# zkonduit/ezkl

Hardware: NVIDIA H100
Metric: prove_time_s (lower is better)
Workload: dtype u32 limbs (254-bit Montgomery integers mod BN254 r/p)

## Files before the change

ezkl_b200/csrc/msm.cu:

```cuda
#include "msm.cuh"
#include "ec_coop.cuh"

namespace b200 {

static constexpr int HEAVY_CHUNKS = 32;
static constexpr int REDUCE_M_MAX = 32;
static constexpr int TREE_THREADS = 256;

int msm_default_window(size_t n) {
    int k = 0;
    while (((size_t)1 << (k + 1)) <= n) ++k;
    int c = k <= 10 ? 8 : (k <= 13 ? k - 2 : (k <= 17 ? k - 1 : (k <= 19 ? 17 : (k <= 21 ? 18 : 20))));
    if (c < 4) c = 4;
    if (c > 22) c = 22;
    return c;
}

__global__ void __launch_bounds__(128) k_table_next_level(const G1Affine* __restrict__ prev, G1Affine* __restrict__ next, size_t n, int c) {
    size_t i = (size_t)blockIdx.x * blockDim.x + threadIdx.x;
    if (i >= n) return;
    G1Affine p = prev[i];
    G1Xyzz a = g1_dbl_affine(p);
#pragma unroll 1
    for (int j = 1; j < c; ++j) a = g1_dbl(a);
    next[i] = g1_to_affine(a);
}

int msm_table_build(MsmTable* t, const G1Affine* d_bases, size_t n, int c, cudaStream_t st) {
    B200_CHECK(n > 0, -1, "msm_table_build: empty base vector");
    if (c <= 0) c = msm_default_window(n);
    int W = (255 + c - 1) / c;
    B200_CHECK((size_t)W * n < ((size_t)1 << 31), -1, "msm_table_build: W*n = %zu exceeds the 31-bit entry index", (size_t)W * n);
    t->n = n; t->c = c; t->W = W;
    B200_CUDA(cudaGetDevice(&t->device));
    B200_CUDA(cudaMalloc(&t->d_table, sizeof(G1Affine) * n * W));
    B200_CUDA(cudaMemcpyAsync(t->d_table, d_bases, sizeof(G1Affine) * n, cudaMemcpyDeviceToDevice, st));
    for (int w = 1; w < W; ++w) {
        k_table_next_level<<<div_up(n, 128), 128, 0, st>>>(t->d_table + (size_t)(w - 1) * n, t->d_table + (size_t)w * n, n, c); count_launch();
    }
    B200_CUDA(cudaGetLastError());
    return 0;
}
void msm_table_free(MsmTable* t) {
    if (t->d_table) cudaFree(t->d_table);
    t->d_table = nullptr;
}

template <bool SCATTER>
__global__ void __launch_bounds__(256) k_digits(const Fr* __restrict__ scalars, size_t stride, uint32_t n, uint32_t table_n, uint32_t base_off, int c, int W,
                                                 uint32_t nbuckets, uint32_t* __restrict__ counters ,
                                                 const uint32_t* __restrict__ offs , uint32_t* __restrict__ ents, size_t ent_stride,
                                                 const uint32_t* __restrict__ skew) {
    const uint32_t col = blockIdx.y;
    const bool aggregate = !SCATTER || skew[col] != 0;
    const Fr* sc = scalars + (size_t)col * stride;
    uint32_t* cnt = counters + (size_t)col * nbuckets;
    const uint32_t* off = SCATTER ? offs + (size_t)col * (nbuckets + 1) : nullptr;
    uint32_t* ent = SCATTER ? ents + (size_t)col * ent_stride : nullptr;
    const unsigned lane = threadIdx.x & 31;
    const uint32_t n_up = (n + 31u) & ~31u;
    for (uint32_t i = blockIdx.x * blockDim.x + threadIdx.x; i < n_up; i += gridDim.x * blockDim.x) {
        const bool valid = i < n;
        Fr s = fp_zero<FrTag>();
        if (valid) s = fp_from_mont(fp_load(sc + i));
        uint32_t carry = 0;
#pragma unroll 1
        for (int w = 0; w < W; ++w) {
            int32_t d = msm_next_digit(s.l, c, &carry);
            const bool nz = d != 0;
            const unsigned act = __ballot_sync(0xffffffffu, nz);
            if (nz && !aggregate) {
                const uint32_t bucket = (uint32_t)(d < 0 ? -d : d) - 1u;
                ent[off[bucket] + atomicAdd(&cnt[bucket], 1u)] = ((uint32_t)w * table_n + base_off + i) | (d < 0 ? 0x80000000u : 0u);
            } else if (nz) {
                const uint32_t bucket = (uint32_t)(d < 0 ? -d : d) - 1u;
                const unsigned peers = __match_any_sync(act, bucket);
                const int leader = __ffs(peers) - 1;
                uint32_t base = 0;
                if ((int)lane == leader) base = atomicAdd(&cnt[bucket], (uint32_t)__popc(peers));
                if (SCATTER) {
                    base = __shfl_sync(peers, base, leader);
                    const uint32_t rank = __popc(peers & ((1u << lane) - 1u));
                    ent[off[bucket] + base + rank] = ((uint32_t)w * table_n + base_off + i) | (d < 0 ? 0x80000000u : 0u);
                }
            }
        }
    }
}

__global__ void __launch_bounds__(1024) k_scan_buckets(const uint32_t* __restrict__ counts, uint32_t* __restrict__ offs, uint32_t* __restrict__ chunk_offs,
                                                        uint32_t nbuckets, uint32_t cap, uint32_t* __restrict__ skew ) {
    __shared__ uint32_t sh_max;
    if (threadIdx.x == 0) sh_max = 0;
    __syncthreads();
    const uint32_t col = blockIdx.x;
    const uint32_t lc = 31u - (uint32_t)__clz(cap);
    const uint32_t* cnt = counts + (size_t)col * nbuckets;
    uint32_t* off = offs + (size_t)col * (nbuckets + 1);
    uint32_t* coff = chunk_offs + (size_t)col * (nbuckets + 1);
    const uint32_t ipt = (nbuckets + blockDim.x - 1) / blockDim.x;
    const uint32_t lo = threadIdx.x * ipt, hi = min(lo + ipt, nbuckets);
    uint32_t s = 0, cs = 0;
    uint32_t mx = 0;
    const bool vec = (ipt & 3u) == 0 && lo + ipt <= nbuckets;
    if (vec) {
        const uint4* c4 = reinterpret_cast<const uint4*>(cnt + lo);
#pragma unroll 4
        for (uint32_t q = 0; q < (ipt >> 2); ++q) {
            const uint4 v = c4[q];
            s += v.x + v.y + v.z + v.w;
            cs += ((v.x + cap - 1) >> lc) + ((v.y + cap - 1) >> lc) + ((v.z + cap - 1) >> lc) + ((v.w + cap - 1) >> lc);
            mx = max(max(mx, v.x), max(max(v.y, v.z), v.w));
        }
    } else {
        for (uint32_t b = lo; b < hi; ++b) { uint32_t v = cnt[b]; s += v; cs += ((v + cap - 1) >> lc); mx = max(mx, v); }
    }
    if (mx) atomicMax(&sh_max, mx);
    uint32_t tot, ctot;
    uint32_t ex = block_exclusive_scan(s, &tot);
    uint32_t cex = block_exclusive_scan(cs, &ctot);
    if (vec) {
        const uint4* c4 = reinterpret_cast<const uint4*>(cnt + lo);
#pragma unroll 4
        for (uint32_t q = 0; q < (ipt >> 2); ++q) {
            const uint4 v = c4[q];
            const uint32_t b = lo + 4 * q;
            off[b] = ex; coff[b] = cex; ex += v.x; cex += ((v.x + cap - 1) >> lc);
            off[b + 1] = ex; coff[b + 1] = cex; ex += v.y; cex += ((v.y + cap - 1) >> lc);
            off[b + 2] = ex; coff[b + 2] = cex; ex += v.z; cex += ((v.z + cap - 1) >> lc);
            off[b + 3] = ex; coff[b + 3] = cex; ex += v.w; cex += ((v.w + cap - 1) >> lc);
        }
    } else {
        for (uint32_t b = lo; b < hi; ++b) { uint32_t v = cnt[b]; off[b] = ex; coff[b] = cex; ex += v; cex += ((v + cap - 1) >> lc); }
    }
    if (threadIdx.x == 0) {
        off[nbuckets] = tot; coff[nbuckets] = ctot;
        skew[col] = sh_max > 16u * (tot / nbuckets + 1u) ? 1u : 0u;
    }
}

__global__ void __launch_bounds__(256) k_fill_chunks(const uint32_t* __restrict__ offs, const uint32_t* __restrict__ chunk_offs, uint32_t nbuckets, uint32_t cap,
                                                      uint32_t* __restrict__ chunk_start, uint32_t* __restrict__ chunk_len, size_t chunk_stride,
                                                      uint32_t* __restrict__ len_hist , uint32_t* __restrict__ heavy , uint32_t heavy_stride) {
    extern __shared__ uint32_t sh_hist[];
    const uint32_t col = blockIdx.y;
    for (uint32_t j = threadIdx.x; j <= cap; j += blockDim.x) sh_hist[j] = 0;
    __syncthreads();
    const uint32_t* off = offs + (size_t)col * (nbuckets + 1);
    const uint32_t* coff = chunk_offs + (size_t)col * (nbuckets + 1);
    uint32_t* cs = chunk_start + (size_t)col * chunk_stride;
    uint32_t* cl = chunk_len + (size_t)col * chunk_stride;
    const uint32_t b = blockIdx.x * blockDim.x + threadIdx.x;
    if (b < nbuckets) {
        const uint32_t start = off[b], size = off[b + 1] - start, c0 = coff[b], nch = coff[b + 1] - c0;
        for (uint32_t j = 0; j < nch; ++j) {
            const uint32_t len = min(cap, size - j * cap);
            cs[c0 + j] = start + j * cap;
            cl[c0 + j] = len;
            if (j + 1 == nch) atomicAdd(&sh_hist[len], 1u);
        }
        if (nch > 1) atomicAdd(&sh_hist[cap], nch - 1);
        if (nch > (uint32_t)HEAVY_CHUNKS) {
            uint32_t* hv = heavy + (size_t)col * heavy_stride;
            uint32_t slot = atomicAdd(&hv[0], 1u);
            if (slot + 1 < heavy_stride) hv[1 + slot] = b;
        }
    }
    __syncthreads();
    uint32_t* gh = len_hist + (size_t)col * (cap + 1);
    for (uint32_t j = threadIdx.x; j <= cap; j += blockDim.x) if (sh_hist[j]) atomicAdd(&gh[j], sh_hist[j]);
}

__global__ void k_len_offsets(const uint32_t* __restrict__ len_hist, uint32_t* __restrict__ len_offs, uint32_t cap) {
    const uint32_t col = blockIdx.x;
    if (threadIdx.x != 0) return;
    const uint32_t* h = len_hist + (size_t)col * (cap + 1);
    uint32_t* o = len_offs + (size_t)col * (cap + 1);
    uint32_t acc = 0;
    for (int l = (int)cap; l >= 0; --l) { o[l] = acc; acc += h[l]; }
}

__global__ void __launch_bounds__(256) k_order_chunks(const uint32_t* __restrict__ chunk_len, size_t chunk_stride, const uint32_t* __restrict__ chunk_offs, uint32_t nbuckets,
                                                       const uint32_t* __restrict__ len_offs, uint32_t* __restrict__ len_cursor, uint32_t cap, uint32_t* __restrict__ order) {
    const uint32_t col = blockIdx.y;
    const uint32_t nchunks = chunk_offs[(size_t)col * (nbuckets + 1) + nbuckets];
    const uint32_t* cl = chunk_len + (size_t)col * chunk_stride;
    uint32_t* ord = order + (size_t)col * chunk_stride;
    const uint32_t* lo = len_offs + (size_t)col * (cap + 1);
    uint32_t* lc = len_cursor + (size_t)col * (cap + 1);
    const unsigned lane = threadIdx.x & 31;
    const uint32_t n_up = (nchunks + 31u) & ~31u;
    for (uint32_t i = blockIdx.x * blockDim.x + threadIdx.x; i < n_up; i += gridDim.x * blockDim.x) {
        const bool valid = i < nchunks;
        const uint32_t len = valid ? cl[i] : 0;
        const unsigned act = __ballot_sync(0xffffffffu, valid);
        if (valid) {
            const unsigned peers = __match_any_sync(act, len);
            const int leader = __ffs(peers) - 1;
            uint32_t base = 0;
            if ((int)lane == leader) base = atomicAdd(&lc[len], (uint32_t)__popc(peers));
            base = __shfl_sync(peers, base, leader);
            ord[lo[len] + base + __popc(peers & ((1u << lane) - 1u))] = i;
        }
    }
}

DEV G1Affine load_base(const G1Affine* __restrict__ table, uint32_t e) {
    const uint4* q = reinterpret_cast<const uint4*>(table + (e & 0x7fffffffu));
    uint4 a = __ldg(q), b = __ldg(q + 1), c = __ldg(q + 2), d = __ldg(q + 3);
    G1Affine p;
    p.x.l[0] = a.x; p.x.l[1] = a.y; p.x.l[2] = a.z; p.x.l[3] = a.w; p.x.l[4] = b.x; p.x.l[5] = b.y; p.x.l[6] = b.z; p.x.l[7] = b.w;
    p.y.l[0] = c.x; p.y.l[1] = c.y; p.y.l[2] = c.z; p.y.l[3] = c.w; p.y.l[4] = d.x; p.y.l[5] = d.y; p.y.l[6] = d.z; p.y.l[7] = d.w;
    return p;
}
__global__ void __launch_bounds__(128, 4) k_accumulate(const G1Affine* __restrict__ table, const uint32_t* __restrict__ ents, size_t ent_stride,
                                                        const uint32_t* __restrict__ chunk_start, const uint32_t* __restrict__ chunk_len, const uint32_t* __restrict__ order,
                                                        size_t chunk_stride, const uint32_t* __restrict__ chunk_offs, uint32_t nbuckets, G1Xyzz* __restrict__ chunk_sums) {
    const uint32_t col = blockIdx.y;
    const uint32_t nchunks = chunk_offs[(size_t)col * (nbuckets + 1) + nbuckets];
    const uint32_t* ent = ents + (size_t)col * ent_stride;
    for (uint32_t t = blockIdx.x * blockDim.x + threadIdx.x; t < nchunks; t += gridDim.x * blockDim.x) {
        const uint32_t ch = order[(size_t)col * chunk_stride + t];
        const uint32_t start = chunk_start[(size_t)col * chunk_stride + ch], len = chunk_len[(size_t)col * chunk_stride + ch];
        uint32_t e = ent[start];
        G1Affine p = load_base(table, e);
        if (e >> 31) p = g1_neg(p);
        G1Xyzz acc = g1_to_xyzz(p);
        if (len > 1) {
            uint32_t e_next = ent[start + 1];
            G1Affine nx = load_base(table, e_next);
#pragma unroll 1
            for (uint32_t j = 1; j < len; ++j) {
                p = nx; e = e_next;
                if (j + 1 < len) { e_next = ent[start + j + 1]; nx = load_base(table, e_next); }
                if (e >> 31) p = g1_neg(p);
                acc = g1_add_mixed(acc, p);
            }
        }
        chunk_sums[(size_t)col * chunk_stride + ch] = acc;
    }
}

DEV G1Xyzz block_sum(G1Xyzz v, G1Xyzz* sh) {
    sh[threadIdx.x] = v;
    __syncthreads();
#pragma unroll 1
    for (unsigned s = blockDim.x / 2; s > 0; s >>= 1) {
        if (threadIdx.x < s) { v = g1_add(v, sh[threadIdx.x + s]); sh[threadIdx.x] = v; }
        __syncthreads();
    }
    return v;
}

__global__ void __launch_bounds__(128) k_combine(const uint32_t* __restrict__ chunk_offs, uint32_t nbuckets, const G1Xyzz* __restrict__ chunk_sums, size_t chunk_stride,
                                                  G1Xyzz* __restrict__ bucket_sums) {
    const uint32_t col = blockIdx.y;
    const uint32_t b = blockIdx.x * blockDim.x + threadIdx.x;
    if (b >= nbuckets) return;
    const uint32_t* coff = chunk_offs + (size_t)col * (nbuckets + 1);
    const uint32_t c0 = coff[b], nch = coff[b + 1] - c0;
    if (nch > (uint32_t)HEAVY_CHUNKS) return;
    const G1Xyzz* cs = chunk_sums + (size_t)col * chunk_stride;
    G1Xyzz acc = g1_xyzz_identity();
    if (nch > 0) acc = cs[c0];
#pragma unroll 1
    for (uint32_t j = 1; j < nch; ++j) acc = g1_add(acc, cs[c0 + j]);
    bucket_sums[(size_t)col * nbuckets + b] = acc;
}
__global__ void __launch_bounds__(TREE_THREADS) k_combine_heavy(const uint32_t* __restrict__ heavy, uint32_t heavy_stride, const uint32_t* __restrict__ chunk_offs, uint32_t nbuckets,
                                                                 const G1Xyzz* __restrict__ chunk_sums, size_t chunk_stride, G1Xyzz* __restrict__ bucket_sums) {
    __shared__ G1Xyzz sh[TREE_THREADS];
    const uint32_t col = blockIdx.y;
    const uint32_t* hv = heavy + (size_t)col * heavy_stride;
    const uint32_t nheavy = min(hv[0], heavy_stride - 1);
    const uint32_t* coff = chunk_offs + (size_t)col * (nbuckets + 1);
    const G1Xyzz* cs = chunk_sums + (size_t)col * chunk_stride;
    for (uint32_t h = blockIdx.x; h < nheavy; h += gridDim.x) {
        const uint32_t b = hv[1 + h];
        const uint32_t c0 = coff[b], nch = coff[b + 1] - c0;
        G1Xyzz acc = g1_xyzz_identity();
#pragma unroll 1
        for (uint32_t j = threadIdx.x; j < nch; j += TREE_THREADS) acc = g1_add(acc, cs[c0 + j]);
        acc = block_sum(acc, sh);
        if (threadIdx.x == 0) bucket_sums[(size_t)col * nbuckets + b] = acc;
        __syncthreads();
    }
}

template <int MIN_CTAS>
__global__ void __launch_bounds__(TREE_THREADS, MIN_CTAS) k_reduce(const G1Xyzz* __restrict__ bucket_sums, uint32_t nbuckets, G1Xyzz* __restrict__ partials, uint32_t nparts, uint32_t per_thread) {
    __shared__ G1Xyzz sh[TREE_THREADS];
    const uint32_t col = blockIdx.y;
    const G1Xyzz* bs = bucket_sums + (size_t)col * nbuckets;
    const uint32_t t = blockIdx.x * blockDim.x + threadIdx.x;
    const uint32_t lo = t * per_thread;
    G1Xyzz run = g1_xyzz_identity(), acc = g1_xyzz_identity();
    if (lo < nbuckets) {
        const uint32_t hi = min(lo + per_thread, nbuckets);
#pragma unroll 1
        for (uint32_t b = hi; b-- > lo;) {
            run = g1_add(run, bs[b]);
            acc = g1_add(acc, run);
        }
        if (lo > 0) acc = g1_add(acc, g1_mul_small(run, lo));
    }
    acc = block_sum(acc, sh);
    if (threadIdx.x == 0) partials[(size_t)col * nparts + blockIdx.x] = acc;
}
__global__ void __launch_bounds__(TREE_THREADS) k_final(const G1Xyzz* __restrict__ partials, uint32_t nparts, G1Xyzz* __restrict__ out) {
    __shared__ G1Xyzz sh[TREE_THREADS];
    const uint32_t col = blockIdx.x;
    G1Xyzz acc = g1_xyzz_identity();
#pragma unroll 1
    for (uint32_t j = threadIdx.x; j < nparts; j += blockDim.x) acc = g1_add(acc, partials[(size_t)col * nparts + j]);
    acc = block_sum(acc, sh);
    if (threadIdx.x == 0) out[col] = acc;
}

static constexpr int COOP_LT = TREE_THREADS / 4;
static constexpr size_t COOP_MAX_BUCKETS = (size_t)3 << 15;
DEV G1Xyzz block_sum_coop(G1Xyzz v, G1Xyzz* sh) {
    const unsigned lt = threadIdx.x >> 2, q = threadIdx.x & 3;
    if (q == 0) sh[lt] = v;
    __syncthreads();
#pragma unroll 1
    for (unsigned s = COOP_LT / 2; s > 0; s >>= 1) {
        if (lt < s) { v = g1_add_coop4(v, sh[lt + s]); if (q == 0) sh[lt] = v; }
        __syncthreads();
    }
    return v;
}
__global__ void __launch_bounds__(TREE_THREADS) k_reduce_coop(const G1Xyzz* __restrict__ bucket_sums, uint32_t nbuckets, G1Xyzz* __restrict__ partials, uint32_t nparts, uint32_t per_thread) {
    __shared__ G1Xyzz sh[COOP_LT];
    const uint32_t col = blockIdx.y;
    const G1Xyzz* bs = bucket_sums + (size_t)col * nbuckets;
    const uint32_t t = blockIdx.x * COOP_LT + (threadIdx.x >> 2);
    const uint32_t lo = t * per_thread;
    G1Xyzz run = g1_xyzz_identity(), acc = g1_xyzz_identity();
    if (lo < nbuckets) {
        const uint32_t hi = min(lo + per_thread, nbuckets);
#pragma unroll 1
        for (uint32_t b = hi; b-- > lo;) {
            run = g1_add_coop4(run, bs[b]);
            acc = g1_add_coop4(acc, run);
        }
        if (lo > 0) acc = g1_add_coop4(acc, g1_mul_small_coop4(run, lo));
    }
    acc = block_sum_coop(acc, sh);
    if (threadIdx.x == 0) partials[(size_t)col * nparts + blockIdx.x] = acc;
}
__global__ void __launch_bounds__(TREE_THREADS) k_final_coop(const G1Xyzz* __restrict__ partials, uint32_t nparts, G1Xyzz* __restrict__ out) {
    __shared__ G1Xyzz sh[COOP_LT];
    const uint32_t col = blockIdx.x;
    G1Xyzz acc = g1_xyzz_identity();
#pragma unroll 1
    for (uint32_t j = threadIdx.x >> 2; j < nparts; j += COOP_LT) acc = g1_add_coop4(acc, partials[(size_t)col * nparts + j]);
    acc = block_sum_coop(acc, sh);
    if (threadIdx.x == 0) out[col] = acc;
}

__global__ void __launch_bounds__(128) k_g1_generate(uint64_t seed, size_t n, G1Affine* __restrict__ out) {
    const size_t i = (size_t)blockIdx.x * blockDim.x + threadIdx.x;
    if (i >= n) return;
    uint32_t s[8];
    uint64_t z = seed + 0x9e3779b97f4a7c15ull * (uint64_t)(i + 1);
#pragma unroll
    for (int w = 0; w < 4; ++w) {
        z += 0x9e3779b97f4a7c15ull;
        uint64_t x = z; x = (x ^ (x >> 30)) * 0xbf58476d1ce4e5b9ull; x = (x ^ (x >> 27)) * 0x94d049bb133111ebull; x ^= x >> 31;
        s[2 * w] = (uint32_t)x; s[2 * w + 1] = (uint32_t)(x >> 32);
    }
    s[7] &= 0x0fffffffu;
    G1Affine g; g.x = fp_one<FqTag>(); g.y = fp_one<FqTag>() + fp_one<FqTag>();
    G1Xyzz acc = g1_xyzz_identity();
#pragma unroll 1
    for (int b = 251; b >= 0; --b) {
        acc = g1_dbl(acc);
        if ((s[b >> 5] >> (b & 31)) & 1) acc = g1_add_mixed(acc, g);
    }
    out[i] = g1_to_affine(acc);
}
int g1_generate_run(uint64_t seed, size_t n, G1Affine* d_out, cudaStream_t st) {
    if (n == 0) return 0;
    k_g1_generate<<<div_up(n, 128), 128, 0, st>>>(seed, n, d_out); count_launch();
    B200_CUDA(cudaGetLastError());
    return 0;
}

__global__ void __launch_bounds__(128) k_g1_fixed_base_mul(const Fr* __restrict__ scalars, size_t n, G1Affine base, G1Affine* __restrict__ out) {
    const size_t i = (size_t)blockIdx.x * blockDim.x + threadIdx.x;
    if (i >= n) return;
    const Fr s = fp_from_mont(fp_load(scalars + i));
    G1Xyzz acc = g1_xyzz_identity();
#pragma unroll 1
    for (int b = 253; b >= 0; --b) {
        acc = g1_dbl(acc);
        if ((s.l[b >> 5] >> (b & 31)) & 1) acc = g1_add_mixed(acc, base);
    }
    out[i] = g1_to_affine(acc);
}
int g1_fixed_base_mul_run(const Fr* d_scalars, size_t n, const G1Affine& base, G1Affine* d_out, cudaStream_t st) {
    if (n == 0) return 0;
    k_g1_fixed_base_mul<<<div_up(n, 128), 128, 0, st>>>(d_scalars, n, base, d_out); count_launch();
    B200_CUDA(cudaGetLastError());
    return 0;
}

int g1_sum_run(const G1Xyzz* d_points, size_t groups, size_t count, G1Xyzz* d_out, cudaStream_t st) {
    if (groups == 0) return 0;
    B200_CHECK(groups <= 0x7fffffffu && count <= 0xffffffffu, -1, "g1_sum: sizes out of range");
    k_final_coop<<<(unsigned)groups, TREE_THREADS, 0, st>>>(d_points, (uint32_t)count, d_out); count_launch();
    B200_CUDA(cudaGetLastError());
    return 0;
}

static uint32_t pick_cap(size_t total_entries) {
    size_t target = total_entries / ((size_t)sm_count() * 512 * 4);
    uint32_t cap = 16;
    while (cap < 512 && cap < target) cap <<= 1;
    return cap;
}

size_t msm_workspace_per_column(const MsmTable& t, size_t n) {
    const size_t nb = (size_t)1 << (t.c - 1), ents = n * t.W;
    const size_t chunk_stride = nb + ents / 16 + 1;
    return ents * 4 + chunk_stride * (12 + sizeof(G1Xyzz)) + nb * (sizeof(G1Xyzz) + 24) + 65536;
}

int msm_run(const MsmTable& t, const Fr* d_scalars, size_t n, size_t stride, int batch, G1Xyzz* d_out, MsmWorkspace& ws, cudaStream_t st, size_t base_off) {
    B200_CHECK(base_off + n <= t.n, -1, "msm: pairs [%zu, %zu) but only %zu bases registered", base_off, base_off + n, t.n);
    B200_CHECK(batch > 0 && batch <= 65535, -1, "msm: batch %d out of range", batch);
    if (n == 0) {
        B200_CUDA(cudaMemsetAsync(d_out, 0, sizeof(G1Xyzz) * batch, st));
        return 0;
    }
    const int c = t.c, W = t.W;
    const uint32_t nb = 1u << (c - 1);
    const size_t ent_stride = (size_t)n * W;
    B200_CHECK(ent_stride < ((size_t)1 << 32), -1, "msm: n*W too large");
    const Config& cfg = config();
    const uint32_t cap = pick_cap(ent_stride * batch);
    const size_t chunk_stride = (size_t)nb + ent_stride / cap + 1;
    const uint32_t heavy_stride = (uint32_t)(ent_stride / ((size_t)cap * HEAVY_CHUNKS)) + 2;
    const size_t all_buckets = (size_t)batch * nb;
    uint32_t reduce_m = REDUCE_M_MAX, reduce_threads = TREE_THREADS;
    if (all_buckets <= ((size_t)1 << 15)) { reduce_m = 4; reduce_threads = 128; }
    else if (all_buckets <= ((size_t)1 << 18)) { reduce_m = 8; reduce_threads = 128; }
    else if (all_buckets <= ((size_t)5 << 17)) { reduce_m = 16; reduce_threads = 256; }
    else if (all_buckets < ((size_t)37 << 15)) { reduce_m = 32; reduce_threads = 128; }
    while (reduce_m > 1 && reduce_m > nb) reduce_m >>= 1;
    if (cfg.msm_reduce_m >= 1 && cfg.msm_reduce_m <= 4096) reduce_m = (uint32_t)cfg.msm_reduce_m;
    if (cfg.msm_reduce_threads == 32 || cfg.msm_reduce_threads == 64 || cfg.msm_reduce_threads == 128 || cfg.msm_reduce_threads == 256) reduce_threads = (uint32_t)cfg.msm_reduce_threads;
    const bool coop = cfg.msm_reduce2 == 2 && all_buckets <= COOP_MAX_BUCKETS;
    if (coop) { reduce_m = cfg.msm_reduce_m >= 1 ? reduce_m : 8; reduce_threads = TREE_THREADS; }
    const uint32_t nparts = div_up(div_up(nb, reduce_m), coop ? COOP_LT : reduce_threads);
    uint32_t final_threads = 32;
    while (final_threads < (uint32_t)TREE_THREADS && final_threads < nparts) final_threads <<= 1;

    const size_t n_hist = (size_t)batch * nb, n_len = (size_t)batch * (cap + 1), n_heavy = (size_t)batch * heavy_stride;
    const size_t counts_words = 2 * n_hist + 2 * n_len + n_heavy;
    if (ws.counts.ensure(counts_words * 4)) return -2;
    uint32_t* hist = ws.counts.as<uint32_t>();
    uint32_t* cursor = hist + n_hist;
    uint32_t* len_hist = cursor + n_hist;
    uint32_t* len_cursor = len_hist + n_len;
    uint32_t* heavy = len_cursor + n_len;
    const size_t n_off = (size_t)batch * (nb + 1);
    if (ws.offs.ensure((2 * n_off + n_len + (size_t)batch) * 4)) return -2;
    uint32_t* offs = ws.offs.as<uint32_t>();
    uint32_t* chunk_offs = offs + n_off;
    uint32_t* len_offs = chunk_offs + n_off;
    uint32_t* skew = len_offs + n_len;
    if (ws.ents.ensure((size_t)batch * ent_stride * 4)) return -2;
    uint32_t* ents = ws.ents.as<uint32_t>();
    if (ws.subs.ensure((size_t)batch * chunk_stride * 4 * 3)) return -2;
    uint32_t* chunk_start = ws.subs.as<uint32_t>();
    uint32_t* chunk_len = chunk_start + (size_t)batch * chunk_stride;
    uint32_t* order = chunk_len + (size_t)batch * chunk_stride;
    if (ws.sums.ensure(sizeof(G1Xyzz) * ((size_t)batch * chunk_stride + (size_t)batch * nb + (size_t)batch * nparts))) return -2;
    G1Xyzz* chunk_sums = ws.sums.as<G1Xyzz>();
    G1Xyzz* bucket_sums = chunk_sums + (size_t)batch * chunk_stride;
    G1Xyzz* partials = bucket_sums + (size_t)batch * nb;

    ProfScope ps_total(PROF_MSM_TOTAL, st);
    B200_CUDA(cudaMemsetAsync(hist, 0, counts_words * 4, st));
    if (prof_enabled()) prof_mark(PROF_MSM_RECODE, st, true);
    const unsigned sms = (unsigned)sm_count();
    const unsigned dig_blocks = min(div_up(n, 256), sms * 8u);
    dim3 gd(dig_blocks, batch);
    k_digits<false><<<gd, 256, 0, st>>>(d_scalars, stride, (uint32_t)n, (uint32_t)t.n, (uint32_t)base_off, c, W, nb, hist, nullptr, nullptr, 0, nullptr); count_launch();
    k_scan_buckets<<<batch, 1024, 0, st>>>(hist, offs, chunk_offs, nb, cap, skew); count_launch();
    k_digits<true><<<gd, 256, 0, st>>>(d_scalars, stride, (uint32_t)n, (uint32_t)t.n, (uint32_t)base_off, c, W, nb, cursor, offs, ents, ent_stride, skew); count_launch();
    k_fill_chunks<<<dim3(div_up(nb, 256), batch), 256, (cap + 1) * 4, st>>>(offs, chunk_offs, nb, cap, chunk_start, chunk_len, chunk_stride, len_hist, heavy, heavy_stride); count_launch();
    k_len_offsets<<<batch, 32, 0, st>>>(len_hist, len_offs, cap); count_launch();
    const unsigned ch_blocks = min(div_up(chunk_stride, 256), sms * 8u);
    k_order_chunks<<<dim3(ch_blocks, batch), 256, 0, st>>>(chunk_len, chunk_stride, chunk_offs, nb, len_offs, len_cursor, cap, order); count_launch();
    if (prof_enabled()) prof_mark(PROF_MSM_RECODE, st, false);
    const unsigned acc_blocks = min(div_up(chunk_stride, 128), sms * 16u);
    {
        ProfScope ps(PROF_MSM_ACCUMULATE, st);
        k_accumulate<<<dim3(acc_blocks, batch), 128, 0, st>>>(t.d_table, ents, ent_stride, chunk_start, chunk_len, order, chunk_stride, chunk_offs, nb, chunk_sums); count_launch();
    }
    ProfScope ps_tail(PROF_MSM_TAIL, st);
    k_combine<<<dim3(div_up(nb, 128), batch), 128, 0, st>>>(chunk_offs, nb, chunk_sums, chunk_stride, bucket_sums); count_launch();
    k_combine_heavy<<<dim3(32, batch), TREE_THREADS, 0, st>>>(heavy, heavy_stride, chunk_offs, nb, chunk_sums, chunk_stride, bucket_sums); count_launch();
    if (coop) {
        k_reduce_coop<<<dim3(nparts, batch), TREE_THREADS, 0, st>>>(bucket_sums, nb, partials, nparts, reduce_m); count_launch();
        k_final_coop<<<batch, TREE_THREADS, 0, st>>>(partials, nparts, d_out); count_launch();
    } else {
        k_reduce<1><<<dim3(nparts, batch), reduce_threads, 0, st>>>(bucket_sums, nb, partials, nparts, reduce_m); count_launch();
        k_final<<<batch, final_threads, 0, st>>>(partials, nparts, d_out); count_launch();
    }
    B200_CUDA(cudaGetLastError());
    return 0;
}

}
```

Before: 0.08930.

## Replace atomic bucket scatter with two-level tiled radix sort for MSM recoding

Replaces the count/scan/scatter of signed digits into buckets, which used global atomics, with a two-pass radix sort. Coarse bins are tiled in shared memory with per-tile counts and scans. A per-bin fine sort in shared memory then produces bucket-ordered entries, chunk metadata and the length histogram. Digit loops also exit early once a warp's scalars are exhausted. The aim is to cut scattered global atomics and uncoalesced writes, at the cost of more kernels, temporary buffers aliased onto the sums workspace, and more complex geometry logic.

```diff
diff --git a/ezkl_b200/csrc/msm.cu b/ezkl_b200/csrc/msm.cu
--- a/ezkl_b200/csrc/msm.cu
+++ b/ezkl_b200/csrc/msm.cu
@@ -46,162 +46,315 @@
     t->d_table = nullptr;
 }
 
-template <bool SCATTER>
-__global__ void __launch_bounds__(256) k_digits(const Fr* __restrict__ scalars, size_t stride, uint32_t n, uint32_t table_n, uint32_t base_off, int c, int W,
-                                                 uint32_t nbuckets, uint32_t* __restrict__ counters ,
-                                                 const uint32_t* __restrict__ offs , uint32_t* __restrict__ ents, size_t ent_stride,
-                                                 const uint32_t* __restrict__ skew) {
-    const uint32_t col = blockIdx.y;
-    const bool aggregate = !SCATTER || skew[col] != 0;
+static constexpr int BIN_THREADS = 256;
+static constexpr uint32_t BIN_TILE_ENTS = 8192;
+static constexpr int FINE_THREADS = 512, FINE_ITEMS = 10;
+static constexpr uint32_t FINE_TILE = FINE_THREADS * FINE_ITEMS;
+static constexpr int FINE_BITS_MAX = 13;
+static constexpr int FINE_STREAM = 8;
+static_assert(FINE_TILE <= 65536, "k_fine_sort packs a rank below FINE_TILE into 16 bits");
+
+DEV uint32_t smem_rank(uint32_t* cnt, uint32_t key, bool valid) {
+    const unsigned lane = threadIdx.x & 31;
+    const unsigned act = __ballot_sync(0xffffffffu, valid);
+    if (act == 0) return 0;
+    const int lead = __ffs(act) - 1;
+    const uint32_t k0 = __shfl_sync(0xffffffffu, key, lead);
+    const bool mine = valid && key == k0;
+    const unsigned peers = __ballot_sync(0xffffffffu, mine);
+    uint32_t base = 0;
+    if ((int)lane == lead) base = atomicAdd(&cnt[k0], (uint32_t)__popc(peers));
+    base = __shfl_sync(0xffffffffu, base, lead);
+    if (mine) return base + __popc(peers & ((1u << lane) - 1u));
+    return valid ? atomicAdd(&cnt[key], 1u) : 0u;
+}
+
+DEV uint32_t scan_array(const uint32_t* a, uint32_t* out, uint32_t m) {
+    const uint32_t per = (m + blockDim.x - 1) / blockDim.x, lo = min(threadIdx.x * per, m), hi = min(lo + per, m);
+    uint32_t s = 0;
+    for (uint32_t j = lo; j < hi; ++j) s += a[j];
+    uint32_t tot;
+    uint32_t ex = block_exclusive_scan(s, &tot);
+    for (uint32_t j = lo; j < hi; ++j) { const uint32_t v = a[j]; out[j] = ex; ex += v; }
+    return tot;
+}
+
+DEV bool warp_digits_done(const uint32_t s[8], uint32_t carry) {
+    const uint32_t rest = s[0] | s[1] | s[2] | s[3] | s[4] | s[5] | s[6] | s[7] | carry;
+    return __all_sync(0xffffffffu, rest == 0);
+}
+
+DEV uint32_t block_sum_u32(const uint32_t* a, uint32_t m) {
+    uint32_t s = 0, tot;
+    for (uint32_t j = threadIdx.x; j < m; j += blockDim.x) s += a[j];
+    block_exclusive_scan(s, &tot);
+    return tot;
+}
+
+struct BinGeom {
+    uint32_t n, table_n, base_off;
+    int c, W;
+    uint32_t tile;
+    uint32_t ntiles;
+    int fb;
+    uint32_t nbins;
+};
+
+__global__ void __launch_bounds__(BIN_THREADS) k_bin_count(const Fr* __restrict__ scalars, size_t stride, BinGeom g, uint32_t* __restrict__ counts) {
+    extern __shared__ uint32_t sh_cnt[];
+    const uint32_t col = blockIdx.y, tile = blockIdx.x;
+    for (uint32_t b = threadIdx.x; b < g.nbins; b += blockDim.x) sh_cnt[b] = 0;
+    __syncthreads();
     const Fr* sc = scalars + (size_t)col * stride;
-    uint32_t* cnt = counters + (size_t)col * nbuckets;
-    const uint32_t* off = SCATTER ? offs + (size_t)col * (nbuckets + 1) : nullptr;
-    uint32_t* ent = SCATTER ? ents + (size_t)col * ent_stride : nullptr;
-    const unsigned lane = threadIdx.x & 31;
-    const uint32_t n_up = (n + 31u) & ~31u;
-    for (uint32_t i = blockIdx.x * blockDim.x + threadIdx.x; i < n_up; i += gridDim.x * blockDim.x) {
-        const bool valid = i < n;
+    for (uint32_t j0 = 0; j0 < g.tile; j0 += BIN_THREADS) {
+        const uint32_t j = j0 + threadIdx.x, i = tile * g.tile + j;
+        const bool valid = j < g.tile && i < g.n;
         Fr s = fp_zero<FrTag>();
         if (valid) s = fp_from_mont(fp_load(sc + i));
         uint32_t carry = 0;
 #pragma unroll 1
-        for (int w = 0; w < W; ++w) {
-            int32_t d = msm_next_digit(s.l, c, &carry);
-            const bool nz = d != 0;
-            const unsigned act = __ballot_sync(0xffffffffu, nz);
-            if (nz && !aggregate) {
-                const uint32_t bucket = (uint32_t)(d < 0 ? -d : d) - 1u;
-                ent[off[bucket] + atomicAdd(&cnt[bucket], 1u)] = ((uint32_t)w * table_n + base_off + i) | (d < 0 ? 0x80000000u : 0u);
-            } else if (nz) {
-                const uint32_t bucket = (uint32_t)(d < 0 ? -d : d) - 1u;
-                const unsigned peers = __match_any_sync(act, bucket);
-                const int leader = __ffs(peers) - 1;
-                uint32_t base = 0;
-                if ((int)lane == leader) base = atomicAdd(&cnt[bucket], (uint32_t)__popc(peers));
-                if (SCATTER) {
-                    base = __shfl_sync(peers, base, leader);
-                    const uint32_t rank = __popc(peers & ((1u << lane) - 1u));
-                    ent[off[bucket] + base + rank] = ((uint32_t)w * table_n + base_off + i) | (d < 0 ? 0x80000000u : 0u);
-                }
+        for (int w = 0; w < g.W && !warp_digits_done(s.l, carry); ++w) {
+            const int32_t d = msm_next_digit(s.l, g.c, &carry);
+            const uint32_t bucket = (uint32_t)(d < 0 ? -d : d) - 1u;
+            smem_rank(sh_cnt, bucket >> g.fb, d != 0);
+        }
+    }
+    __syncthreads();
+    uint32_t* cnt = counts + (size_t)col * g.nbins * g.ntiles;
+    for (uint32_t b = threadIdx.x; b < g.nbins; b += blockDim.x) cnt[(size_t)b * g.ntiles + tile] = sh_cnt[b];
+}
+
+__global__ void __launch_bounds__(256) k_bin_scan(const uint32_t* __restrict__ counts, uint32_t* __restrict__ bin_offs, uint32_t* __restrict__ bin_tot, BinGeom g) {
+    const uint32_t col = blockIdx.y, bin = blockIdx.x;
+    const size_t at = ((size_t)col * g.nbins + bin) * g.ntiles;
+    const uint32_t tot = scan_array(counts + at, bin_offs + at, g.ntiles);
+    if (threadIdx.x == 0) bin_tot[(size_t)col * g.nbins + bin] = tot;
+}
+
+__global__ void __launch_bounds__(BIN_THREADS) k_bin_scatter(const Fr* __restrict__ scalars, size_t stride, BinGeom g, const uint32_t* __restrict__ counts,
+                                                              const uint32_t* __restrict__ bin_offs, const uint32_t* __restrict__ bin_tot, uint32_t* __restrict__ bin_start,
+                                                              uint32_t* __restrict__ tmp_e, uint16_t* __restrict__ tmp_k, size_t ent_stride) {
+    extern __shared__ uint32_t sh[];
+    uint32_t* loff = sh;
+    uint32_t* cur = loff + g.nbins;
+    uint32_t* gdst = cur + g.nbins;
+    uint32_t* se = gdst + g.nbins;
+    uint16_t* sk = reinterpret_cast<uint16_t*>(se + BIN_TILE_ENTS);
+    uint16_t* sb = sk + BIN_TILE_ENTS;
+    const uint32_t col = blockIdx.y, tile = blockIdx.x;
+    const size_t m = (size_t)g.nbins * g.ntiles;
+    const uint32_t* cnt = counts + (size_t)col * m;
+    const uint32_t* bo = bin_offs + (size_t)col * m;
+    const uint32_t* bt = bin_tot + (size_t)col * g.nbins;
+    for (uint32_t b = threadIdx.x; b < g.nbins; b += blockDim.x) { loff[b] = cnt[(size_t)b * g.ntiles + tile]; cur[b] = 0; gdst[b] = bt[b]; }
+    __syncthreads();
+    const uint32_t total = scan_array(loff, loff, g.nbins);
+    scan_array(gdst, gdst, g.nbins);
+    __syncthreads();
+    for (uint32_t b = threadIdx.x; b < g.nbins; b += blockDim.x) {
+        if (tile == 0) bin_start[(size_t)col * g.nbins + b] = gdst[b];
+        gdst[b] += bo[(size_t)b * g.ntiles + tile] - loff[b];
+    }
+    const Fr* sc = scalars + (size_t)col * stride;
+    const uint32_t fmask = (1u << g.fb) - 1u;
+    for (uint32_t j0 = 0; j0 < g.tile; j0 += BIN_THREADS) {
+        const uint32_t j = j0 + threadIdx.x, i = tile * g.tile + j;
+        const bool valid = j < g.tile && i < g.n;
+        Fr s = fp_zero<FrTag>();
+        if (valid) s = fp_from_mont(fp_load(sc + i));
+        uint32_t carry = 0;
+#pragma unroll 1
+        for (int w = 0; w < g.W && !warp_digits_done(s.l, carry); ++w) {
+            const int32_t d = msm_next_digit(s.l, g.c, &carry);
+            const uint32_t bucket = (uint32_t)(d < 0 ? -d : d) - 1u, bin = bucket >> g.fb;
+            const uint32_t r = smem_rank(cur, bin, d != 0);
+            if (d != 0) {
+                const uint32_t p = loff[bin] + r;
+                se[p] = ((uint32_t)w * g.table_n + g.base_off + i) | (d < 0 ? 0x80000000u : 0u);
+                sk[p] = (uint16_t)(bucket & fmask);
+                sb[p] = (uint16_t)bin;
             }
         }
     }
-}
-
-__global__ void __launch_bounds__(1024) k_scan_buckets(const uint32_t* __restrict__ counts, uint32_t* __restrict__ offs, uint32_t* __restrict__ chunk_offs,
-                                                        uint32_t nbuckets, uint32_t cap, uint32_t* __restrict__ skew ) {
-    __shared__ uint32_t sh_max;
-    if (threadIdx.x == 0) sh_max = 0;
-    __syncthreads();
+    __syncthreads();
+    uint32_t* te = tmp_e + (size_t)col * ent_stride;
+    uint16_t* tk = tmp_k + (size_t)col * ent_stride;
+    for (uint32_t p = threadIdx.x; p < total; p += blockDim.x) {
+        const uint32_t d = gdst[sb[p]] + p;
+        te[d] = se[p];
+        tk[d] = sk[p];
+    }
+}
+
+__global__ void __launch_bounds__(FINE_THREADS, 2) k_fine_sort(const uint32_t* __restrict__ tmp_e, const uint16_t* __restrict__ tmp_k, size_t ent_stride,
+                                                               const uint32_t* __restrict__ bin_start, const uint32_t* __restrict__ bin_tot, BinGeom g, uint32_t cap,
+                                                               uint32_t* __restrict__ ents,
+                                                               uint32_t* __restrict__ offs , uint32_t* __restrict__ bin_chunks ,
+                                                               uint32_t* __restrict__ len_hist ) {
+    extern __shared__ uint32_t sh[];
+    const uint32_t nf = 1u << g.fb;
+    uint32_t* gh = sh;
+    uint32_t* cur = gh + nf;
+    uint32_t* lh = cur + nf;
+    uint32_t* loff = lh + nf;
+    uint32_t* lens = loff + nf;
+    uint32_t* oe = lens + cap + 1;
+    const uint32_t col = blockIdx.y, bin = blockIdx.x;
+    const uint32_t lo = bin_start[(size_t)col * g.nbins + bin], size = bin_tot[(size_t)col * g.nbins + bin];
+    const uint32_t* te = tmp_e + (size_t)col * ent_stride + lo;
+    const uint16_t* tk = tmp_k + (size_t)col * ent_stride + lo;
+    uint32_t* out = ents + (size_t)col * ent_stride + lo;
+    for (uint32_t f = threadIdx.x; f < nf; f += blockDim.x) { gh[f] = 0; lh[f] = 0; cur[f] = 0; }
+    for (uint32_t l = threadIdx.x; l <= cap; l += blockDim.x) lens[l] = 0;
+    __syncthreads();
+    if (size <= FINE_TILE) {
+        uint32_t e[FINE_ITEMS], k[FINE_ITEMS];
+#pragma unroll
+        for (int it = 0; it < FINE_ITEMS; ++it) {
+            const uint32_t p = it * FINE_THREADS + threadIdx.x;
+            const bool v = p < size;
+            e[it] = v ? te[p] : 0u;
+            k[it] = v ? tk[p] : 0u;
+        }
+#pragma unroll
+        for (int it = 0; it < FINE_ITEMS; ++it) k[it] |= smem_rank(lh, k[it], it * FINE_THREADS + threadIdx.x < size) << 16;
+        __syncthreads();
+        scan_array(lh, loff, nf);
+        __syncthreads();
+#pragma unroll
+        for (int it = 0; it < FINE_ITEMS; ++it)
+            if (it * FINE_THREADS + threadIdx.x < size) oe[loff[k[it] & 0xffffu] + (k[it] >> 16)] = e[it];
+        for (uint32_t f = threadIdx.x; f < nf; f += blockDim.x) { gh[f] = lh[f]; cur[f] = loff[f] + lh[f]; }
+        __syncthreads();
+        for (uint32_t p = threadIdx.x; p < size; p += blockDim.x) out[p] = oe[p];
+    } else {
+        for (uint32_t p0 = 0; p0 < size; p0 += FINE_STREAM * FINE_THREADS) {
+            uint32_t k[FINE_STREAM];
+#pragma unroll
+            for (int q = 0; q < FINE_STREAM; ++q) {
+                const uint32_t p = p0 + q * FINE_THREADS + threadIdx.x;
+                k[q] = p < size ? tk[p] : 0u;
+            }
+#pragma unroll
+            for (int q = 0; q < FINE_STREAM; ++q) smem_rank(gh, k[q], p0 + q * FINE_THREADS + threadIdx.x < size);
+        }
+        __syncthreads();
+        scan_array(gh, cur, nf);
+        __syncthreads();
+        for (uint32_t p0 = 0; p0 < size; p0 += FINE_STREAM * FINE_THREADS) {
+            uint32_t e[FINE_STREAM], k[FINE_STREAM];
+#pragma unroll
+            for (int q = 0; q < FINE_STREAM; ++q) {
+                const uint32_t p = p0 + q * FINE_THREADS + threadIdx.x;
+                e[q] = p < size ? te[p] : 0u;
+                k[q] = p < size ? tk[p] : 0u;
+            }
+#pragma unroll
+            for (int q = 0; q < FINE_STREAM; ++q) {
+                const bool v = p0 + q * FINE_THREADS + threadIdx.x < size;
+                const uint32_t d = smem_rank(cur, k[q], v);
+                if (v) out[d] = e[q];
+            }
+        }
+    }
+    __syncthreads();
+    const uint32_t lc = 31u - (uint32_t)__clz(cap);
+    uint32_t* off = offs + (size_t)col * ((size_t)(g.nbins << g.fb) + 1) + ((size_t)bin << g.fb);
+    uint32_t nch_sum = 0;
+    for (uint32_t f = threadIdx.x; f < nf; f += blockDim.x) {
+        const uint32_t cnt = gh[f];
+        off[f] = lo + cur[f] - cnt;
+        const uint32_t nch = (cnt + cap - 1) >> lc;
+        nch_sum += nch;
+        if (nch) {
+            atomicAdd(&lens[cnt - (nch - 1) * cap], 1u);
+            if (nch > 1) atomicAdd(&lens[cap], nch - 1);
+        }
+    }
+    uint32_t tot;
+    block_exclusive_scan(nch_sum, &tot);
+    if (threadIdx.x == 0) bin_chunks[(size_t)col * g.nbins + bin] = tot;
+    uint32_t* lhg = len_hist + (size_t)col * (cap + 1);
+    for (uint32_t l = threadIdx.x; l <= cap; l += blockDim.x) if (lens[l]) atomicAdd(&lhg[l], lens[l]);
+}
+
+__global__ void __launch_bounds__(1024) k_chunk_scan(uint32_t* __restrict__ bin_chunks, const uint32_t* __restrict__ bin_tot, BinGeom g, uint32_t nb,
+                                                      uint32_t* __restrict__ offs, uint32_t* __restrict__ chunk_offs, const uint32_t* __restrict__ len_hist,
+                                                      uint32_t* __restrict__ len_offs, uint32_t cap) {
     const uint32_t col = blockIdx.x;
+    uint32_t* bc = bin_chunks + (size_t)col * g.nbins;
+    const uint32_t tot = scan_array(bc, bc, g.nbins);
+    const uint32_t ents = block_sum_u32(bin_tot + (size_t)col * g.nbins, g.nbins);
+    if (threadIdx.x == 0) {
+        chunk_offs[(size_t)col * (nb + 1) + nb] = tot;
+        offs[(size_t)col * (nb + 1) + nb] = ents;
+    }
+    const uint32_t j = threadIdx.x, l = cap - j;
+    const uint32_t v = j <= cap ? len_hist[(size_t)col * (cap + 1) + l] : 0u;
+    uint32_t all;
+    const uint32_t ex = block_exclusive_scan(v, &all);
+    if (j <= cap) len_offs[(size_t)col * (cap + 1) + l] = ex;
+}
+
+__global__ void __launch_bounds__(256) k_chunk_fill(const uint32_t* __restrict__ offs, const uint32_t* __restrict__ bin_chunks, BinGeom g, uint32_t nb, uint32_t cap,
+                                                     uint32_t* __restrict__ chunk_offs, uint32_t* __restrict__ chunk_start, uint32_t* __restrict__ chunk_len, size_t chunk_stride,
+                                                     const uint32_t* __restrict__ len_offs, uint32_t* __restrict__ len_cursor, uint32_t* __restrict__ order,
+                                                     uint32_t* __restrict__ heavy , uint32_t heavy_stride) {
+    extern __shared__ uint32_t sh[];
+    uint32_t* lcnt = sh;
+    uint32_t* lbase = lcnt + cap + 1;
+    const uint32_t col = blockIdx.y, bin = blockIdx.x, nf = 1u << g.fb, b0 = bin << g.fb;
     const uint32_t lc = 31u - (uint32_t)__clz(cap);
-    const uint32_t* cnt = counts + (size_t)col * nbuckets;
-    uint32_t* off = offs + (size_t)col * (nbuckets + 1);
-    uint32_t* coff = chunk_offs + (size_t)col * (nbuckets + 1);
-    const uint32_t ipt = (nbuckets + blockDim.x - 1) / blockDim.x;
-    const uint32_t lo = threadIdx.x * ipt, hi = min(lo + ipt, nbuckets);
-    uint32_t s = 0, cs = 0;
-    uint32_t mx = 0;
-    const bool vec = (ipt & 3u) == 0 && lo + ipt <= nbuckets;
-    if (vec) {
-        const uint4* c4 = reinterpret_cast<const uint4*>(cnt + lo);
-#pragma unroll 4
-        for (uint32_t q = 0; q < (ipt >> 2); ++q) {
-            const uint4 v = c4[q];
-            s += v.x + v.y + v.z + v.w;
-            cs += ((v.x + cap - 1) >> lc) + ((v.y + cap - 1) >> lc) + ((v.z + cap - 1) >> lc) + ((v.w + cap - 1) >> lc);
-            mx = max(max(mx, v.x), max(max(v.y, v.z), v.w));
-        }
-    } else {
-        for (uint32_t b = lo; b < hi; ++b) { uint32_t v = cnt[b]; s += v; cs += ((v + cap - 1) >> lc); mx = max(mx, v); }
-    }
-    if (mx) atomicMax(&sh_max, mx);
-    uint32_t tot, ctot;
-    uint32_t ex = block_exclusive_scan(s, &tot);
-    uint32_t cex = block_exclusive_scan(cs, &ctot);
-    if (vec) {
-        const uint4* c4 = reinterpret_cast<const uint4*>(cnt + lo);
-#pragma unroll 4
-        for (uint32_t q = 0; q < (ipt >> 2); ++q) {
-            const uint4 v = c4[q];
-            const uint32_t b = lo + 4 * q;
-            off[b] = ex; coff[b] = cex; ex += v.x; cex += ((v.x + cap - 1) >> lc);
-            off[b + 1] = ex; coff[b + 1] = cex; ex += v.y; cex += ((v.y + cap - 1) >> lc);
-            off[b + 2] = ex; coff[b + 2] = cex; ex += v.z; cex += ((v.z + cap - 1) >> lc);
-            off[b + 3] = ex; coff[b + 3] = cex; ex += v.w; cex += ((v.w + cap - 1) >> lc);
-        }
-    } else {
-        for (uint32_t b = lo; b < hi; ++b) { uint32_t v = cnt[b]; off[b] = ex; coff[b] = cex; ex += v; cex += ((v + cap - 1) >> lc); }
-    }
-    if (threadIdx.x == 0) {
-        off[nbuckets] = tot; coff[nbuckets] = ctot;
-        skew[col] = sh_max > 16u * (tot / nbuckets + 1u) ? 1u : 0u;
-    }
-}
-
-__global__ void __launch_bounds__(256) k_fill_chunks(const uint32_t* __restrict__ offs, const uint32_t* __restrict__ chunk_offs, uint32_t nbuckets, uint32_t cap,
-                                                      uint32_t* __restrict__ chunk_start, uint32_t* __restrict__ chunk_len, size_t chunk_stride,
-                                                      uint32_t* __restrict__ len_hist , uint32_t* __restrict__ heavy , uint32_t heavy_stride) {
-    extern __shared__ uint32_t sh_hist[];
-    const uint32_t col = blockIdx.y;
-    for (uint32_t j = threadIdx.x; j <= cap; j += blockDim.x) sh_hist[j] = 0;
-    __syncthreads();
-    const uint32_t* off = offs + (size_t)col * (nbuckets + 1);
-    const uint32_t* coff = chunk_offs + (size_t)col * (nbuckets + 1);
+    const uint32_t* off = offs + (size_t)col * (nb + 1);
+    uint32_t* coff = chunk_offs + (size_t)col * (nb + 1);
     uint32_t* cs = chunk_start + (size_t)col * chunk_stride;
     uint32_t* cl = chunk_len + (size_t)col * chunk_stride;
-    const uint32_t b = blockIdx.x * blockDim.x + threadIdx.x;
-    if (b < nbuckets) {
-        const uint32_t start = off[b], size = off[b + 1] - start, c0 = coff[b], nch = coff[b + 1] - c0;
+    uint32_t* ord = order + (size_t)col * chunk_stride;
+    for (uint32_t l = threadIdx.x; l <= cap; l += blockDim.x) lcnt[l] = 0;
+    const uint32_t per = (nf + blockDim.x - 1) / blockDim.x, flo = min(threadIdx.x * per, nf), fhi = min(flo + per, nf);
+    uint32_t s = 0;
+    for (uint32_t f = flo; f < fhi; ++f) s += (off[b0 + f + 1] - off[b0 + f] + cap - 1) >> lc;
+    uint32_t tot;
+    const uint32_t c_first = bin_chunks[(size_t)col * g.nbins + bin] + block_exclusive_scan(s, &tot);
+    uint32_t c0 = c_first;
+    for (uint32_t f = flo; f < fhi; ++f) {
+        const uint32_t b = b0 + f, start = off[b], size = off[b + 1] - start, nch = (size + cap - 1) >> lc;
+        coff[b] = c0;
         for (uint32_t j = 0; j < nch; ++j) {
-            const uint32_t len = min(cap, size - j * cap);
             cs[c0 + j] = start + j * cap;
-            cl[c0 + j] = len;
-            if (j + 1 == nch) atomicAdd(&sh_hist[len], 1u);
-        }
-        if (nch > 1) atomicAdd(&sh_hist[cap], nch - 1);
+            cl[c0 + j] = min(cap, size - j * cap);
+        }
+        if (nch) {
+            atomicAdd(&lcnt[size - (nch - 1) * cap], 1u);
+            if (nch > 1) atomicAdd(&lcnt[cap], nch - 1);
+        }
         if (nch > (uint32_t)HEAVY_CHUNKS) {
             uint32_t* hv = heavy + (size_t)col * heavy_stride;
-            uint32_t slot = atomicAdd(&hv[0], 1u);
+            const uint32_t slot = atomicAdd(&hv[0], 1u);
             if (slot + 1 < heavy_stride) hv[1 + slot] = b;
         }
-    }
-    __syncthreads();
-    uint32_t* gh = len_hist + (size_t)col * (cap + 1);
-    for (uint32_t j = threadIdx.x; j <= cap; j += blockDim.x) if (sh_hist[j]) atomicAdd(&gh[j], sh_hist[j]);
-}
-
-__global__ void k_len_offsets(const uint32_t* __restrict__ len_hist, uint32_t* __restrict__ len_offs, uint32_t cap) {
-    const uint32_t col = blockIdx.x;
-    if (threadIdx.x != 0) return;
-    const uint32_t* h = len_hist + (size_t)col * (cap + 1);
-    uint32_t* o = len_offs + (size_t)col * (cap + 1);
-    uint32_t acc = 0;
-    for (int l = (int)cap; l >= 0; --l) { o[l] = acc; acc += h[l]; }
-}
-
-__global__ void __launch_bounds__(256) k_order_chunks(const uint32_t* __restrict__ chunk_len, size_t chunk_stride, const uint32_t* __restrict__ chunk_offs, uint32_t nbuckets,
-                                                       const uint32_t* __restrict__ len_offs, uint32_t* __restrict__ len_cursor, uint32_t cap, uint32_t* __restrict__ order) {
-    const uint32_t col = blockIdx.y;
-    const uint32_t nchunks = chunk_offs[(size_t)col * (nbuckets + 1) + nbuckets];
-    const uint32_t* cl = chunk_len + (size_t)col * chunk_stride;
-    uint32_t* ord = order + (size_t)col * chunk_stride;
+        c0 += nch;
+    }
+    __syncthreads();
     const uint32_t* lo = len_offs + (size_t)col * (cap + 1);
-    uint32_t* lc = len_cursor + (size_t)col * (cap + 1);
-    const unsigned lane = threadIdx.x & 31;
-    const uint32_t n_up = (nchunks + 31u) & ~31u;
-    for (uint32_t i = blockIdx.x * blockDim.x + threadIdx.x; i < n_up; i += gridDim.x * blockDim.x) {
-        const bool valid = i < nchunks;
-        const uint32_t len = valid ? cl[i] : 0;
-        const unsigned act = __ballot_sync(0xffffffffu, valid);
-        if (valid) {
-            const unsigned peers = __match_any_sync(act, len);
-            const int leader = __ffs(peers) - 1;
-            uint32_t base = 0;
-            if ((int)lane == leader) base = atomicAdd(&lc[len], (uint32_t)__popc(peers));
-            base = __shfl_sync(peers, base, leader);
-            ord[lo[len] + base + __popc(peers & ((1u << lane) - 1u))] = i;
-        }
+    uint32_t* lcur = len_cursor + (size_t)col * (cap + 1);
+    for (uint32_t l = threadIdx.x; l <= cap; l += blockDim.x) {
+        if (lcnt[l]) lbase[l] = lo[l] + atomicAdd(&lcur[l], lcnt[l]);
+        lcnt[l] = 0;
+    }
+    __syncthreads();
+    c0 = c_first;
+    for (uint32_t f = flo; f < fhi; ++f) {
+        const uint32_t b = b0 + f, size = off[b + 1] - off[b], nch = (size + cap - 1) >> lc;
+        if (nch > 1) {
+            const uint32_t r = atomicAdd(&lcnt[cap], nch - 1);
+            for (uint32_t j = 0; j + 1 < nch; ++j) ord[lbase[cap] + r + j] = c0 + j;
+        }
+        if (nch) {
+            const uint32_t last = size - (nch - 1) * cap;
+            ord[lbase[last] + atomicAdd(&lcnt[last], 1u)] = c0 + nch - 1;
+        }
+        c0 += nch;
     }
 }
 
@@ -421,10 +574,24 @@
     return cap;
 }
 
+static BinGeom bin_geom(const MsmTable& t, size_t n) {
+    BinGeom g{};
+    g.n = (uint32_t)n; g.table_n = (uint32_t)t.n; g.c = t.c; g.W = t.W;
+    g.tile = 1;
+    while (g.tile * 2 * (uint32_t)t.W <= BIN_TILE_ENTS) g.tile <<= 1;
+    g.ntiles = div_up(n, g.tile);
+    const size_t ents = n * (size_t)t.W;
+    int cb = t.c - 1 > FINE_BITS_MAX ? t.c - 1 - FINE_BITS_MAX : 0;
+    while (cb < t.c - 1 && ((size_t)3 * FINE_TILE << cb) < 4 * ents && ((size_t)8 << (cb + 1)) <= (size_t)g.tile * t.W) ++cb;
+    g.fb = t.c - 1 - cb;
+    g.nbins = 1u << cb;
+    return g;
+}
+
 size_t msm_workspace_per_column(const MsmTable& t, size_t n) {
     const size_t nb = (size_t)1 << (t.c - 1), ents = n * t.W;
     const size_t chunk_stride = nb + ents / 16 + 1;
-    return ents * 4 + chunk_stride * (12 + sizeof(G1Xyzz)) + nb * (sizeof(G1Xyzz) + 24) + 65536;
+    return ents * 4 + chunk_stride * (12 + sizeof(G1Xyzz)) + nb * (sizeof(G1Xyzz) + 8) + ents / 128 + 65536;
 }
 
 int msm_run(const MsmTable& t, const Fr* d_scalars, size_t n, size_t stride, int batch, G1Xyzz* d_out, MsmWorkspace& ws, cudaStream_t st, size_t base_off) {
@@ -457,44 +624,58 @@
     uint32_t final_threads = 32;
     while (final_threads < (uint32_t)TREE_THREADS && final_threads < nparts) final_threads <<= 1;
 
-    const size_t n_hist = (size_t)batch * nb, n_len = (size_t)batch * (cap + 1), n_heavy = (size_t)batch * heavy_stride;
-    const size_t counts_words = 2 * n_hist + 2 * n_len + n_heavy;
+    const BinGeom g = [&] { BinGeom x = bin_geom(t, n); x.base_off = (uint32_t)base_off; return x; }();
+    B200_CHECK(g.fb <= FINE_BITS_MAX && g.nbins <= 1024, -1, "msm: window %d gives %u coarse bins of %d fine bits", c, g.nbins, g.fb);
+    const size_t n_cnt = (size_t)g.nbins * g.ntiles;
+
+    const size_t n_len = (size_t)batch * (cap + 1), n_heavy = (size_t)batch * heavy_stride;
+    const size_t counts_words = 2 * n_len + n_heavy;
     if (ws.counts.ensure(counts_words * 4)) return -2;
-    uint32_t* hist = ws.counts.as<uint32_t>();
-    uint32_t* cursor = hist + n_hist;
-    uint32_t* len_hist = cursor + n_hist;
+    uint32_t* len_hist = ws.counts.as<uint32_t>();
     uint32_t* len_cursor = len_hist + n_len;
     uint32_t* heavy = len_cursor + n_len;
     const size_t n_off = (size_t)batch * (nb + 1);
-    if (ws.offs.ensure((2 * n_off + n_len + (size_t)batch) * 4)) return -2;
+    if (ws.offs.ensure((2 * n_off + n_len + (size_t)batch * g.nbins) * 4)) return -2;
     uint32_t* offs = ws.offs.as<uint32_t>();
     uint32_t* chunk_offs = offs + n_off;
     uint32_t* len_offs = chunk_offs + n_off;
-    uint32_t* skew = len_offs + n_len;
+    uint32_t* bin_chunks = len_offs + n_len;
     if (ws.ents.ensure((size_t)batch * ent_stride * 4)) return -2;
     uint32_t* ents = ws.ents.as<uint32_t>();
     if (ws.subs.ensure((size_t)batch * chunk_stride * 4 * 3)) return -2;
     uint32_t* chunk_start = ws.subs.as<uint32_t>();
     uint32_t* chunk_len = chunk_start + (size_t)batch * chunk_stride;
     uint32_t* order = chunk_len + (size_t)batch * chunk_stride;
-    if (ws.sums.ensure(sizeof(G1Xyzz) * ((size_t)batch * chunk_stride + (size_t)batch * nb + (size_t)batch * nparts))) return -2;
+    const size_t tmp_e_words = (size_t)batch * ent_stride, tmp_k_words = ((size_t)batch * ent_stride + 1) / 2;
+    const size_t sort_bytes = 4 * (tmp_e_words + tmp_k_words + (size_t)batch * (2 * n_cnt + 2 * g.nbins));
+    const size_t sums_bytes = sizeof(G1Xyzz) * ((size_t)batch * chunk_stride + (size_t)batch * nb + (size_t)batch * nparts);
+    if (ws.sums.ensure(std::max(sums_bytes, sort_bytes))) return -2;
     G1Xyzz* chunk_sums = ws.sums.as<G1Xyzz>();
     G1Xyzz* bucket_sums = chunk_sums + (size_t)batch * chunk_stride;
     G1Xyzz* partials = bucket_sums + (size_t)batch * nb;
+    uint32_t* tmp_e = ws.sums.as<uint32_t>();
+    uint16_t* tmp_k = reinterpret_cast<uint16_t*>(tmp_e + tmp_e_words);
+    uint32_t* bin_counts = tmp_e + tmp_e_words + tmp_k_words;
+    uint32_t* bin_offs = bin_counts + (size_t)batch * n_cnt;
+    uint32_t* bin_tot = bin_offs + (size_t)batch * n_cnt;
+    uint32_t* bin_start = bin_tot + (size_t)batch * g.nbins;
+
+    const size_t scatter_smem = 3 * 4 * (size_t)g.nbins + (size_t)BIN_TILE_ENTS * 8;
+    const size_t fine_smem = 4 * (4 * ((size_t)1 << g.fb) + cap + 1 + (size_t)FINE_TILE);
+    B200_CUDA(cudaFuncSetAttribute(k_bin_scatter, cudaFuncAttributeMaxDynamicSharedMemorySize, (int)scatter_smem));
+    B200_CUDA(cudaFuncSetAttribute(k_fine_sort, cudaFuncAttributeMaxDynamicSharedMemorySize, (int)fine_smem));
 
     ProfScope ps_total(PROF_MSM_TOTAL, st);
-    B200_CUDA(cudaMemsetAsync(hist, 0, counts_words * 4, st));
+    B200_CUDA(cudaMemsetAsync(len_hist, 0, counts_words * 4, st));
     if (prof_enabled()) prof_mark(PROF_MSM_RECODE, st, true);
     const unsigned sms = (unsigned)sm_count();
-    const unsigned dig_blocks = min(div_up(n, 256), sms * 8u);
-    dim3 gd(dig_blocks, batch);
-    k_digits<false><<<gd, 256, 0, st>>>(d_scalars, stride, (uint32_t)n, (uint32_t)t.n, (uint32_t)base_off, c, W, nb, hist, nullptr, nullptr, 0, nullptr); count_launch();
-    k_scan_buckets<<<batch, 1024, 0, st>>>(hist, offs, chunk_offs, nb, cap, skew); count_launch();
-    k_digits<true><<<gd, 256, 0, st>>>(d_scalars, stride, (uint32_t)n, (uint32_t)t.n, (uint32_t)base_off, c, W, nb, cursor, offs, ents, ent_stride, skew); count_launch();
-    k_fill_chunks<<<dim3(div_up(nb, 256), batch), 256, (cap + 1) * 4, st>>>(offs, chunk_offs, nb, cap, chunk_start, chunk_len, chunk_stride, len_hist, heavy, heavy_stride); count_launch();
-    k_len_offsets<<<batch, 32, 0, st>>>(len_hist, len_offs, cap); count_launch();
-    const unsigned ch_blocks = min(div_up(chunk_stride, 256), sms * 8u);
-    k_order_chunks<<<dim3(ch_blocks, batch), 256, 0, st>>>(chunk_len, chunk_stride, chunk_offs, nb, len_offs, len_cursor, cap, order); count_launch();
+    k_bin_count<<<dim3(g.ntiles, batch), BIN_THREADS, g.nbins * 4, st>>>(d_scalars, stride, g, bin_counts); count_launch();
+    k_bin_scan<<<dim3(g.nbins, batch), 256, 0, st>>>(bin_counts, bin_offs, bin_tot, g); count_launch();
+    k_bin_scatter<<<dim3(g.ntiles, batch), BIN_THREADS, scatter_smem, st>>>(d_scalars, stride, g, bin_counts, bin_offs, bin_tot, bin_start, tmp_e, tmp_k, ent_stride); count_launch();
+    k_fine_sort<<<dim3(g.nbins, batch), FINE_THREADS, fine_smem, st>>>(tmp_e, tmp_k, ent_stride, bin_start, bin_tot, g, cap, ents, offs, bin_chunks, len_hist); count_launch();
+    k_chunk_scan<<<batch, 1024, 0, st>>>(bin_chunks, bin_tot, g, nb, offs, chunk_offs, len_hist, len_offs, cap); count_launch();
+    k_chunk_fill<<<dim3(g.nbins, batch), 256, 2 * (cap + 1) * 4, st>>>(offs, bin_chunks, g, nb, cap, chunk_offs, chunk_start, chunk_len, chunk_stride, len_offs, len_cursor,
+                                                                      order, heavy, heavy_stride); count_launch();
     if (prof_enabled()) prof_mark(PROF_MSM_RECODE, st, false);
     const unsigned acc_blocks = min(div_up(chunk_stride, 128), sms * 16u);
     {
```

Result: faster. 0.08453 (median of 6 runs) (-5.3%).
